# kshedden/muscato

Measured on AMD Instinct MI355X. Metric: reads/sec (100 bp, multi-map) at 1/2/4/8 MI355X; confirm-kernel HBM GB/s vs peak, higher is better.
Workload: dtype u32

## Files before the change

muscato_amd/csrc/kernels_common.hpp:

```cpp
#pragma once


#define DEV __device__ __forceinline__
#ifndef MUSC_KERNEL
#define MUSC_KERNEL __global__
#endif
#define READ_HAS_X 0x10000u

DEV uint64_t mix64(uint64_t x) {
  x ^= x >> 33;
  x *= 0xff51afd7ed558ccdULL;
  x ^= x >> 33;
  x *= 0xc4ceb9fe1a85ec53ULL;
  x ^= x >> 33;
  return x;
}

DEV uint32_t block_hash32(uint32_t k, uint32_t b) {
  uint32_t h = b ^ (k * 0x9E3779B9u + 0x7F4A7C15u);
  h ^= h >> 16;
  h *= 0x85EBCA6Bu;
  h ^= h >> 13;
  h *= 0xC2B2AE35u;
  h ^= h >> 16;
// ... 15 lines not shown
  const int nb = 2 * ww;
  uint64_t h = 0, anymask = 0, key0 = 0;
  for (int c = 0; c < nb; c += 64) {
    const int take = nb - c < 64 ? nb - c : 64;
    const uint64_t key = ext64(w, bo + c) & lowmask64(take);
    const uint64_t mk = m ? (ext64(m, bo + c) & lowmask64(take)) : 0ull;
    if (c == 0) key0 = key;
    anymask |= mk;
    h = mix64(h ^ key ^ mix64(mk + 0x9E3779B97F4A7C15ull * (uint64_t)(c + 1)));
  }
  if (direct && anymask == 0) return (uint32_t)(__brevll(key0) >> (64 - nb));
  return (uint32_t)(h >> (64 - bits));
}

DEV void block_add_u64(unsigned long long v, unsigned long long* dst) {
  __shared__ unsigned long long s_acc[16];
  for (int d = 32; d; d >>= 1) v += __shfl_xor(v, d);
  const int wid = threadIdx.x >> 6, nw = (blockDim.x + 63) >> 6;
  if ((threadIdx.x & 63) == 0) s_acc[wid] = v;
  __syncthreads();
  if (threadIdx.x == 0) {
    unsigned long long t = 0;
    for (int w = 0; w < nw; w++) t += s_acc[w];
    if (t) atomicAdd(dst, t);
  }
  __syncthreads();
}

#ifndef MAX_GRID
#define MAX_GRID 4096u
#endif

enum : int {
  CNT_ACCEPTED = 1,
  CNT_HITS = 2,
  CNT_FLAGS = 3,
  CNT_SCRATCH = 4,
  CNT_OVF_BLOCKS = 5,
  CNT_HOT = 6,
  CNT_PASS_WORDS = 8,
  CNT_BATCH = 8,
  CNT_BATCH_WORDS = 8,
  CNT_WORDS = 16,
  MB_WINDOWS = 0,
  MB_CMP = 1,
  MB_CAND = 3,
  MB_OVF = 4,
  MB_SPILL_MAX = 5,
  MB_TUPLES = 6,
  MB_STAGE_MAX = 7,
  SB_WINDOWS = 0,
  SB_CAND = 3,
  SB_PAIRS = 4,
  SB_TWO = 5,
  SB_DESC_MAX = 7,
};
constexpr unsigned long long FLAG_STAGE_OVERRUN = 1;
constexpr unsigned long long FLAG_HITS_OVERRUN = 2;
constexpr unsigned long long FLAG_SPILL_OVERRUN = 4;
constexpr unsigned long long FLAG_SPEC_REFUSED = 8;


DEV uint32_t ascii_code(unsigned char c, uint32_t* isx) {
  const uint32_t a = c == 'A', cc = c == 'C', g = c == 'G', t = c == 'T';
  *isx = !(a | cc | g | t);
  return cc | (g << 1) | (t * 3u);
}

MUSC_KERNEL void k_pack_db_ascii(const unsigned char* __restrict__ s, uint64_t nbases,
                                uint32_t* __restrict__ db2, uint32_t* __restrict__ dbm2,
                                uint64_t nwords, uint32_t* __restrict__ has_x) {
  const uint64_t w = (uint64_t)blockIdx.x * blockDim.x + threadIdx.x;
// ... 266 lines not shown
```

muscato_amd/csrc/kernels_match.hpp:

```cpp
#pragma once

#define CTX_BASES 120
#define CTX_INLINE 3
#define CTX_MAX_W 4
#define CTX_XFLAG 0x80000000u
#define CTX_XMANY 0xFFu
#define CTX_XNONE 0xFFu

struct __attribute__((aligned(128))) CtxBucket {
  uint32_t count;
  uint32_t ovf;
  uint32_t gene[CTX_INLINE];
  uint32_t jx[CTX_INLINE];
  uint32_t ctx[CTX_INLINE][8];
};
static_assert(sizeof(CtxBucket) == 128, "a context bucket is one cache line");

struct CtxEntry {
  uint32_t gene, jx;
  uint32_t ctx[8];
};
static_assert(sizeof(CtxEntry) == 40, "overflow entries are packed");

#define CTXW_BASES 200
// ... 152 lines not shown
          dst[0] = make_uint4(c[0], c[1], c[2], c[3]);
          dst[1] = make_uint4(c[4], c[5], c[6], c[7]);
        } else {
          uint32_t* p = reinterpret_cast<uint32_t*>(Ev) + ctx_entry_word<false>(T[b].ovf + (slot - CTX_INLINE));
          p[0] = gene | xgene;
          p[1] = (uint32_t)jx | xflag;
#pragma unroll
          for (int i = 0; i < 8; i++) p[2 + i] = c[i];
        }
      }
    }
  }
}

MUSC_KERNEL void k_ctx_ovf_count(const CtxBucket* __restrict__ T, uint64_t nb, uint32_t n_inline, uint64_t* __restrict__ tmp) {
  const uint64_t b = (uint64_t)blockIdx.x * blockDim.x + threadIdx.x;
  if (b < nb) {
    const uint32_t c = T[b].count;
    tmp[b] = c > n_inline ? c - n_inline : 0u;
  } else if (b == nb) {
    tmp[b] = 0;
  }
}

MUSC_KERNEL void k_ctx_ovf_set(CtxBucket* __restrict__ T, uint64_t nb, const uint64_t* __restrict__ tmp) {
  const uint64_t b = (uint64_t)blockIdx.x * blockDim.x + threadIdx.x;
  if (b < nb) T[b].ovf = (uint32_t)tmp[b];
}


struct MatchParams {
  int32_t W, ww, min_dinuc, bits, direct, mmtol, apply_mmtol, max_len, CL;
  uint32_t q1zero_mask;
  int32_t reserved0;
  int32_t win[CTX_MAX_W];
  const uint64_t* seq_off;
  const uint32_t* dbm2;
  uint32_t need[CTX_MAX_W];
  uint32_t wm[CTX_MAX_W][CTX_MAX_W][CTXW_WORDS];
  uint32_t lm[CTXW_BASES + 1][CTX_MAX_W][CTXW_WORDS];
};


inline void match_tables(MatchParams& mp) {
  for (int k = 0; k < CTX_MAX_W; k++) {
    mp.need[k] = 0;
    if (k >= mp.W) continue;
    const int sh = 2 * (mp.CL - mp.win[k]);
    mp.need[k] = ((1u << k) - 1u) | (mp.direct ? 0u : (1u << k));
    for (int kk = 0; kk < mp.W; kk++)
      for (int j = 0; j < CTXW_WORDS; j++)
        mp.wm[k][kk][j] = bit_range_mask(sh + 2 * mp.win[kk] - 32 * j, sh + 2 * (mp.win[kk] + mp.ww) - 32 * j);
    for (int len = 0; len <= CTXW_BASES; len++)
      for (int j = 0; j < CTXW_WORDS; j++) mp.lm[len][k][j] = 0x55555555u & bit_range_mask(sh - 32 * j, sh + 2 * len - 32 * j);
  }
}


#ifndef MATCH_SKETCH_BITS
#define MATCH_SKETCH_BITS 10
#endif

DEV bool ctx_fit(uint32_t jx, uint32_t rem16, int q1, int ww, int rlen, uint32_t* zflag) {
  const int left = (int)(jx > 65535u ? 65535u : jx), right = (int)rem16;
  const int tcap = left + right;
  const int lim0 = 100 - ww < tcap ? 100 - ww : tcap;
  const bool fit0 = rlen <= lim0;
  const bool inside = left == 0 ? fit0 : (rlen - q1 <= right);
  *zflag = (uint32_t)(left == q1) & (uint32_t)!fit0;
  return (q1 <= left) & inside;
}

#define REC_LEN(w) ((w) & 0xFFFFu)
#define REC_BUDGET(w) (((w) >> 17) & 0x7Fu)
#define REC_VALID(w) ((w) >> 24)
// ... 90 lines not shown
}

MUSC_KERNEL void k_xpos_check(const uint32_t* __restrict__ rd, const uint32_t* __restrict__ xpos, uint64_t nreads, int rw,
                             const uint16_t* __restrict__ nmiss_tab, uint32_t max_len, uint32_t xmax, uint32_t* __restrict__ bad) {
  const uint64_t i = (uint64_t)blockIdx.x * blockDim.x + threadIdx.x;
  if (i >= nreads) return;
  const uint32_t cnt = XPOS_CNT(xpos[i]);
  if (cnt <= xmax) return;
  const uint32_t len = rd[(i + 1) * rw - 1] & 0xFFFFu;
  const uint32_t budget = len <= max_len ? nmiss_tab[len] : 0xFFFFu;
  if (cnt == 15u || cnt <= budget) atomicOr(bad, 1u);
}

struct XWins { int32_t n, ww, q1[CTX_MAX_W]; };
template <bool WIDE>
__global__ void k_xpos_check_db(const uint32_t* __restrict__ xpos, uint64_t nreads, XWins wn, uint32_t* __restrict__ bad) {
  typedef XPos<WIDE> XP;
  const uint64_t i = (uint64_t)blockIdx.x * blockDim.x + threadIdx.x;
  if (i >= nreads) return;
  const uint32_t w = xpos[i], cnt = XPOS_CNT(w);
  if (!cnt) return;
  bool b = cnt > XP::MAX;
  for (uint32_t q = 0; q < XP::MAX && q < cnt; q++)
    for (int k = 0; k < wn.n; k++) b |= XP::at(w, q) - (uint32_t)wn.q1[k] < (uint32_t)wn.ww;
  if (b) atomicOr(bad, 1u);
}

MUSC_KERNEL __launch_bounds__(256) void k_compact_w(uint32_t nwt, const uint32_t* __restrict__ tbase,
                                                   const uint32_t* __restrict__ tcount2,
                                                   const uint32_t* __restrict__ tpre, const uint4* __restrict__ stage,
                                                   uint4* __restrict__ hits, uint64_t hits_cap,
                                                   unsigned long long* __restrict__ counters) {
  const unsigned long long base = counters[CNT_HITS];
  if (base + tpre[nwt] > hits_cap) {
    if (blockIdx.x == 0 && threadIdx.x == 0) atomicOr(&counters[CNT_FLAGS], FLAG_HITS_OVERRUN);
    return;
  }
  const uint32_t lane = threadIdx.x & 63;
  for (uint32_t wt = blockIdx.x * 4 + (threadIdx.x >> 6); wt < nwt; wt += gridDim.x * 4) {
    const uint32_t m = tcount2[wt];
    const uint4* __restrict__ src = stage + tbase[wt];
    uint4* __restrict__ dst = hits + base + tpre[wt];
    for (uint32_t j = lane; j < m; j += 64) dst[j] = src[j];
  }
}
```

muscato_amd/csrc/kernels_match_lane.hpp:

```cpp
#pragma once
#include "kernels_match_lane_inst.hpp"
#if defined(MUSC_LANE_DBG) && !defined(MUSC_LANE_DBG_SLOTS)
#define MUSC_LANE_DBG_SLOTS 3
#endif

template <int RW, int NW>
DEV void read_image_n(const Rec<RW>& rec, uint32_t sh, uint32_t (&img)[NW]) {
  const uint32_t bs = sh & 31u;
#define MUSC_IMG_W(Q) (((Q) >= 0 && (Q) < RW - 1) ? rec.w[((Q) >= 0 && (Q) < RW - 1) ? (Q) : 0] : 0u)
#define MUSC_IMG_CASE(WO)                                                  \
  case WO:                                                                 \
    _Pragma("unroll") for (int j = 0; j < NW; j++) {                       \
      const uint32_t hi = MUSC_IMG_W(j - WO), lo = MUSC_IMG_W(j - WO - 1); \
      img[j] = bs ? ((hi << bs) | (lo >> (32u - bs))) : hi;                \
    }                                                                      \
    break;
  switch (__builtin_amdgcn_readfirstlane((int)(sh >> 5))) {
    MUSC_IMG_CASE(0) MUSC_IMG_CASE(1) MUSC_IMG_CASE(2) MUSC_IMG_CASE(3)
    MUSC_IMG_CASE(4) MUSC_IMG_CASE(5) MUSC_IMG_CASE(6) MUSC_IMG_CASE(7)
    MUSC_IMG_CASE(8) MUSC_IMG_CASE(9) MUSC_IMG_CASE(10) MUSC_IMG_CASE(11) MUSC_IMG_CASE(12)
    default:
#pragma unroll
      for (int j = 0; j < NW; j++) img[j] = 0u;
      break;
// ... 44 lines not shown
  constexpr bool SPEC = SGm::on;
  static_assert(!SPEC || (SGm::nwin == W && !WIDE && XM == 0 && SGm::ww <= 15), "a specialised instance is built for its geometry's window count, 120-base buckets, no X, a direct table of one-word keys");
  constexpr int S_WW = SGm::ww, S_CL = SGm::CL, S_L = SGm::L, S_MIND = SGm::min_dinuc;
  constexpr int S_WIN[CTX_MAX_W] = {SGm::win[0], SGm::win[1], SGm::win[2], SGm::win[3]};
  if constexpr (SPEC) {
    bool same = mp->ww == S_WW && mp->CL == S_CL && mp->min_dinuc == S_MIND && mp->direct == 1 && mp->bits == 2 * S_WW && mp->W == W;
#pragma unroll
    for (int k = 0; k < W; k++) same = same && mp->win[k] == S_WIN[k] && mp->need[k] == (1u << k) - 1u;
    if (!same) {
      if (threadIdx.x == 0) atomicOr(&counters[CNT_FLAGS], FLAG_SPEC_REFUSED);
      return;
    }
  }
  const int ww = SPEC ? S_WW : mp->ww, CL = SPEC ? S_CL : mp->CL, min_dinuc = SPEC ? S_MIND : mp->min_dinuc,
            direct = SPEC ? 1 : mp->direct, bits = SPEC ? 2 * S_WW : mp->bits;
  const uint32_t q1zero = mp->q1zero_mask;
  int win[W];
#pragma unroll
  for (int k = 0; k < W; k++) win[k] = SPEC ? S_WIN[k] : mp->win[k];
  uint32_t* const s_sketch = s_dyn + 2 * NWAVE * WT * W;
  for (uint32_t t = threadIdx.x; t < CONF_NM; t += TILE) s_nm[t] = t <= (uint32_t)mp->max_len ? nmiss_tab[t] : (uint16_t)0;
  if (block_mode) {
    for (uint32_t t = threadIdx.x; t < 2u * NWAVE * WT * W; t += TILE) s_dyn[t] = 0;
    if (block_mode == 1)
      for (uint32_t t = threadIdx.x; t < (1u << MATCH_SKETCH_BITS); t += TILE) s_sketch[t] = 0;
  }
  s_best[0][threadIdx.x >> 6][threadIdx.x & 63] = 0xFFFFFFFFu;
  s_best[1][threadIdx.x >> 6][threadIdx.x & 63] = 0xFFFFFFFFu;
  if (blockIdx.x == 0 && threadIdx.x == 0) tcount2[(n + WT - 1) / WT] = 0;
  __syncthreads();

  const uint32_t nwt = (n + WT - 1) / WT;
  const uint32_t gw = blockIdx.x * NWAVE + (threadIdx.x >> 6), nw = gridDim.x * NWAVE;
  const uint64_t region = stage_cap / nw, region0 = region * gw;
  const uint64_t sregion = spill_cap / nw / 2, sregion_w = 2 * sregion * gw;
  uint64_t used = 0;
  uint32_t maxspill = 0;
  uint32_t nvalid = 0, ncand = 0, ncmp = 0, novf = 0, nrep = 0;
  const uint32_t mmtol = (uint32_t)mp->mmtol;
  const bool apply = mp->apply_mmtol != 0;

  auto fetch = [&](uint32_t wt, Rec<RW>& rec) __attribute__((always_inline)) {
    const uint32_t i = wt * WT + (opaque(threadIdx.x) & 63);
    rec.load(rd + (r0 + (i < n ? i : 0)) * (uint64_t)RW, RW);
  };
  auto phase_a = [&](uint32_t wt, const Rec<RW>& rec, uint32_t& xw, uint32_t (&bb)[W]) __attribute__((always_inline)) -> uint32_t {
    const uint32_t lane = opaque(threadIdx.x) & 63;
    const bool active = wt * WT + lane < n;
    const int len = (int)rec.len();
    uint32_t valid = 0;
    xw = 0;
    uint32_t xwin = 0;
    if constexpr (RX) {
      if (active && rec.has_x()) xw = rdx[r0 + wt * WT + lane];
      const uint32_t xc = XPOS_CNT(xw);
      if (xc > XP::MAX) xwin = 0xFFFFFFFFu;
#pragma unroll
      for (int k = 0; k < W; k++) {
        const uint32_t q1 = (uint32_t)win[k];
#pragma unroll
        for (int q = 0; q < (int)XP::MAX; q++)
          if ((uint32_t)q < xc && XP::at(xw, q) - q1 < (uint32_t)ww) xwin |= 1u << k;
      }
    }
    if (ww <= 16 && direct) {
      const uint32_t kmask = ww == 16 ? 0xFFFFFFFFu : ((1u << (2 * ww)) - 1u);
#pragma unroll
      for (int k = 0; k < W; k++) {
        const uint32_t q1 = (uint32_t)win[k], q2 = q1 + (uint32_t)ww;
// ... 189 lines not shown
  for (int k = 0; k < W; k++) wc_prev[k] = oc_prev[k] = ovf_prev[k] = 0, bb_prev[k] = WB_NONE;
  uint32_t o_n = 0, o_k = 0, o_seg = 0, o_meta = 0, o_xw = 0;
  Rec<RW> o_rec;
  o_rec.zero();
  u32x4_u o_q[NQ];
  uint32_t o_t[NT];
#pragma unroll
  for (int q = 0; q < NQ; q++) o_q[q] = u32x4_u{0, 0, 0, 0};
#pragma unroll
  for (int q = 0; q < NT; q++) o_t[q] = 0;

  auto rec_of = [&](uint32_t p, uint32_t seg, Rec<RW>& rec) __attribute__((always_inline)) {
    const uint32_t wid = opaque(threadIdx.x) >> 6;
    const uint4* src = reinterpret_cast<const uint4*>(&s_rec[p][wid][seg * RW]);
#pragma unroll
    for (int q = 0; q < RW / 4; q++) {
      const uint4 v = src[q];
      rec.w[4 * q] = v.x; rec.w[4 * q + 1] = v.y; rec.w[4 * q + 2] = v.z; rec.w[4 * q + 3] = v.w;
    }
  };

  auto phase_a_all = [&](uint32_t wt, uint32_t p, const Rec<RW>& rec, uint32_t& meta, uint32_t& xw, uint32_t (&bb)[W]) __attribute__((always_inline)) {
    const uint32_t tid = opaque(threadIdx.x);
    const uint32_t lane = tid & 63, wid = tid >> 6;
    const uint32_t valid = phase_a(wt, rec, xw, bb);
    const uint32_t len = rec.len();
    const uint32_t budget0 = len < CONF_NM ? s_nm[len] : 0u;
    meta = len | ((budget0 > 127u ? 127u : budget0) << 17) | (valid << 24);
    uint4* dst = reinterpret_cast<uint4*>(&s_rec[p][wid][lane * RW]);
#pragma unroll
    for (int q = 0; q < RW / 4; q++) dst[q] = make_uint4(rec.w[4 * q], rec.w[4 * q + 1], rec.w[4 * q + 2], rec.w[4 * q + 3]);
  };

  if (gw < nwt) {
    Rec<RW> rec0;
    fetch(gw, rec0);
    phase_a_all(gw, 0, rec0, meta_cur, xw_cur, bb_cur);
    if (gw + nw < nwt) fetch(gw + nw, rec_nx);
    wave_lds_sync();
    issue_window(bb_cur[0], va, vb);
  }
  uint32_t wt = gw;
  bool have_prev = false;
#ifdef MUSC_LANE_PROF
  unsigned long long pf[12] = {0, 0, 0, 0, 0, 0, 0, 0, 0, 0, 0, 0}, pt0 = __builtin_amdgcn_s_memtime(), pstart = pt0;
  uint32_t pf_tiles = 0;
#define PF(i) { const unsigned long long t_ = __builtin_amdgcn_s_memtime(); pf[i] += t_ - pt0; pt0 = t_; }
#elif defined(MUSC_LANE_MARK)
#define PF(i) asm volatile("; MARK " #i);
#else
#define PF(i)
#endif
  while (wt < nwt || have_prev) {
    const bool have_cur = wt < nwt;
    const uint32_t tid = opaque(threadIdx.x);
    const uint32_t lane = tid & 63, wid = tid >> 6;
    uint32_t* const cnt_l = s_cb[wid];
    uint32_t* const base_l = s_cb[wid] + WT;
    uint4* const line_l = s_line[wid];
    const bool have_next = wt + nw < nwt;

    auto report_any = [&](uint32_t p, uint32_t& nl, uint32_t w, uint32_t gene, uint32_t pos) __attribute__((always_inline)) {
      const bool acc = w != NX_REJECT;
      if (acc && block_mode) atomicAdd(&s_dyn[(p * NWAVE + wid) * WT * W + ((w >> 20) & 15u) * WT + (w >> 24)], 1u);
      const bool rep = acc && !(w & NX_DUP);
      const unsigned long long vote = __ballot(rep);
      if (vote == 0) return;
      const uint32_t below = __builtin_amdgcn_mbcnt_hi((uint32_t)(vote >> 32), __builtin_amdgcn_mbcnt_lo((uint32_t)vote, 0u));
      const uint32_t slot = nl + below;
      nl += (uint32_t)__popcll(vote);
      if (!rep) return;
      atomicMin(&s_best[p][wid][w >> 24], w & 0xFFFFu);
      if (slot < WLIST) {
        s_list[p][wid][slot] = make_uint3(w, gene, pos);
      } else if (slot - WLIST < sregion) {
        spill[sregion_w + p * sregion + (slot - WLIST)] = make_uint4(w, gene, pos, 0u);
      }
    };
    auto entry_compare = [&](uint32_t p, uint32_t& nl, uint32_t ul, uint32_t n_items, uint32_t ek, uint32_t seg, uint32_t meta,
                             uint32_t xw, const Rec<RW>& rec, const u32x4_u (&eq)[NQ], const uint32_t (&et)[NT]) __attribute__((always_inline)) {
#ifdef MUSC_LANE_DBG
      if (MUSC_LANE_DBG & 32) return;
#endif
      const bool have = lane < n_items;
      if (!__any(have)) return;
      const int len = (int)REC_LEN(meta);
      const uint32_t xi = DBX && (eq[0].y & CTX_XFLAG) ? 0x100u | (eq[0].x >> 24) : 0u;
      const uint32_t gene = xi ? eq[0].x & 0xFFFFFFu : eq[0].x, jx = DBX ? eq[0].y & ~CTX_XFLAG : eq[0].y;
      uint32_t c[NW];
#pragma unroll
      for (int j = 0; j < NW; j++) {
        const int wi = j + 2;
        c[j] = wi < 4 * NQ ? (wi % 4 == 0 ? eq[wi / 4].x : wi % 4 == 1 ? eq[wi / 4].y : wi % 4 == 2 ? eq[wi / 4].z : eq[wi / 4].w) : et[wi - 4 * NQ];
// ... 175 lines not shown
        const uint32_t* sp = reinterpret_cast<const uint32_t*>(spill + sregion_w + pp * sregion + (j - WLIST));
        *gene = __hip_atomic_load(sp + 1, __ATOMIC_RELAXED, __HIP_MEMORY_SCOPE_AGENT);
        *pos = __hip_atomic_load(sp + 2, __ATOMIC_RELAXED, __HIP_MEMORY_SCOPE_AGENT);
        return __hip_atomic_load(sp, __ATOMIC_RELAXED, __HIP_MEMORY_SCOPE_AGENT);
      };
      const uint32_t nuse = spill_ok ? nl : (nl < WLIST ? nl : WLIST);
      uint32_t kw = NX_REJECT, kg = 0, kp = 0, ko = 0;
      if (nuse) {
        best_l[lane] = bestr;
        cnt_l[lane] = 0;
        wave_lds_sync();
        if (lane < nuse) {
          const uint32_t w = item(lane, &kg, &kp);
          const uint32_t rl = w >> 24;
          const uint32_t thr = apply ? best_l[rl] + mmtol : 0xFFFFu;
          if ((w & 0xFFFFu) <= thr) {
            kw = w;
            ko = atomicAdd(&cnt_l[rl], 1u);
          }
        }
        for (uint32_t j = 64 + lane; j < nuse; j += 64) {
          uint32_t g, p;
          const uint32_t w = item(j, &g, &p);
          const uint32_t rl = w >> 24;
          const uint32_t thr = apply ? best_l[rl] + mmtol : 0xFFFFu;
          if ((w & 0xFFFFu) <= thr) atomicAdd(&cnt_l[rl], 1u);
        }
        wave_lds_sync();
        cnum += cnt_l[lane];
      }
      const uint32_t inc = wave_scan_incl(cnum);
      const uint32_t total = __builtin_amdgcn_readlane(inc, 63);
      const uint32_t mybase = inc - cnum;
      const uint64_t base = region0 + used;
      const bool fits = spill_ok && used + total <= region;
      if (lane == 0) {
        tbase[wt_prev] = (uint32_t)base;
        tcount2[wt_prev] = fits ? total : 0u;
      }
      if (fits && total) {
        const uint32_t rid = (uint32_t)(r0 + wt_prev * WT + lane);
        if (s0) put_tuple(&stage[base + mybase], rid, k0g_prev, k0p_prev, k0w_prev & 0xFFFFu);
        if (s1) put_tuple(&stage[base + mybase + (s0 ? 1u : 0u)], rid, k1g_prev, k1p_prev, k1w_prev & 0xFFFFu);
        if (nuse) {
          base_l[lane] = mybase + nown;
          wave_lds_sync();
          if (kw != NX_REJECT) {
            const uint32_t rl = kw >> 24;
            put_tuple(&stage[base + base_l[rl] + ko], (uint32_t)(r0 + wt_prev * WT + rl), kg, kp, kw & 0xFFFFu);
          }
          if (nuse > 64) {
            for (uint32_t j = 64 + lane; j < nuse; j += 64) {
              uint32_t g, p;
              const uint32_t w = item(j, &g, &p);
              const uint32_t rl = w >> 24, v = w & 0xFFFFu;
              const uint32_t thr = apply ? best_l[rl] + mmtol : 0xFFFFu;
              if (v > thr) continue;
              const uint32_t ord = atomicAdd(&cnt_l[rl], 0xFFFFFFFFu) - 1u;
              put_tuple(&stage[base + base_l[rl] + ord], (uint32_t)(r0 + wt_prev * WT + rl), g, p, v);
            }
          }
        }
      }
      wave_lds_sync();
      best_l[lane] = 0xFFFFFFFFu;
      used += total;
      nrep += kc_prev < (uint32_t)OWNK ? kc_prev : (uint32_t)OWNK;
      nrep += lane == 0 ? nl : 0u;
// ... 30 lines not shown
        const bool acc = w != NX_REJECT;
        wck += acc ? 1u : 0u;
        const bool rep = acc && !(w & NX_DUP);
        const bool first = OWNK >= 1 && rep && kc == 0, second = OWNK >= 2 && rep && kc == 1, later = rep && kc >= (uint32_t)OWNK;
        k0w = first ? w : k0w; k0g = first ? gene : k0g; k0p = first ? pos : k0p;
        k1w = second ? w : k1w; k1g = second ? gene : k1g; k1p = second ? pos : k1p;
        kc += rep ? 1u : 0u;
        const uint32_t v = w & 0xFFFFu;
        best = rep && v < best ? v : best;
        const unsigned long long vote = __ballot(later);
        if (vote == 0) return;
        const uint32_t below = __builtin_amdgcn_mbcnt_hi((uint32_t)(vote >> 32), __builtin_amdgcn_mbcnt_lo((uint32_t)vote, 0u));
        const uint32_t slot = nlist + below;
        nlist += (uint32_t)__popcll(vote);
        if (!later) return;
        if (slot < WLIST) {
          list_cur[slot] = make_uint3(w, gene, pos);
        } else if (slot - WLIST < sregion) {
          spill[sregion_w + par * sregion + (slot - WLIST)] = make_uint4(w, gene, pos, 0u);
        }
      };

      auto window = [&](auto kc) __attribute__((always_inline)) {
        constexpr int k = decltype(kc)::value;
        const int q1 = win[k];
        const uint32_t sh = 2u * (uint32_t)(CL - q1);
        WinTab tb;
        win_tab(ulen, k, sh, (uint32_t)rlen, tb);
        {
#pragma unroll
          for (int i = 0; i < 8; i++) line_l[i * 64 + lane] = i < 4 ? va[i] : vb[i - 4];
        }
        PF(0)
        if (k == 0 && have_prev) entry_fetch();
        if (W == 1) {
          if (have_prev) finish_prev();
          if (have_next) phase_a_all(wt + nw, par ^ 1u, rec_nx, meta_nx, xw_nx, bb_nx);
          wave_lds_sync();
        }
        if (k + 1 < W) {
          issue_window(bb_cur[k + 1 < W ? k + 1 : 0], va, vb);
        } else {
          if (have_next) issue_window(bb_nx[0], va, vb);
          if (wt + 2 * nw < nwt) fetch(wt + 2 * nw, rec_nx);
        }
        PF(1)
        wave_lds_sync();
        const uint32_t rb = lane * 8u + (((lane >> 1) & 7u) ^ (lane & 1u));
        const uint4 h0 = line_l[rb], h1 = line_l[rb ^ 1u];
        const uint32_t cnt = bb_cur[k] != WB_NONE ? h0.x : 0u;
        ncand += cnt;
        oc[k] = cnt > (uint32_t)NIN ? cnt - (uint32_t)NIN : 0u;
        ovf[k] = h0.y;
        novf += oc[k];
        PF(2)
        if (W > 1 && k == 0 && have_next) phase_a_all(wt + nw, par ^ 1u, rec_nx, meta_nx, xw_nx, bb_nx);
        PF(8)
        if (W > 1 && k == 1 && have_prev) finish_prev();
        if (k + 1 == W) {
          uint32_t pre[W], total = 0;
#pragma unroll
          for (int kk = 0; kk < W; kk++) {
            const uint32_t inc = wave_scan_incl(oc[kk]);
            pre[kk] = total + inc - oc[kk];
            total += (uint32_t)__builtin_amdgcn_readlane((int)inc, 63);
          }
#ifdef MUSC_LANE_DBG
          if (MUSC_LANE_DBG & 4) total = 0;
#endif
          total_cur = total;
          owner_tables(0, oc, ovf, pre);
          o_n = total < (uint32_t)WT ? total : (uint32_t)WT;
          const uint32_t probe = lane < o_n ? (uint32_t)s_own[wid][lane] : 0u;
          o_k = probe >> 6;
          o_seg = probe & 63u;
          o_meta = s_meta[par][wid][o_seg];
          if constexpr (RX) o_xw = s_xp[par][wid][o_seg];
          rec_of(par, o_seg, o_rec);
        }
        wave_lds_sync();
        PF(3)
        uint32_t img[NW], xm[NW];
        {
          Rec<RW> rec;
          rec_of(par, lane, rec);
          read_image_n<RW, NW>(rec, sh, img);
        }
        x_mask(xw_cur, sh, xm);
        if constexpr (!WIDE) {
// ... 55 lines not shown
      if constexpr (W > 2) window(std::integral_constant<int, 2>{});
      if constexpr (W > 3) window(std::integral_constant<int, 3>{});
#ifdef MUSC_LANE_PROF
      pf_tiles++;
#endif
    } else {
      entry_fetch();
      finish_prev();
    }
    wave_lds_sync();
    have_prev = have_cur;
    if (have_cur) {
      wt_prev = wt;
      nlist_prev = nlist;
      best_prev = best;
      kc_prev = kc; k0w_prev = k0w; k0g_prev = k0g; k0p_prev = k0p; k1w_prev = k1w; k1g_prev = k1g; k1p_prev = k1p;
      ulen_prev = ulen;
      total_prev = total_cur;
#pragma unroll
      for (int k = 0; k < W; k++) {
        if constexpr (BB_LDS) {
          const uint32_t ln = opaque(threadIdx.x) & 63;
          s_bbp[wid][k][ln] = bb_cur[k];
          if (block_mode) s_dyn[(par * NWAVE + wid) * WT * W + k * WT + ln] += wc[k];
        } else {
          bb_prev[k] = bb_cur[k];
          wc_prev[k] = wc[k];
        }
        bb_cur[k] = bb_nx[k], oc_prev[k] = oc[k], ovf_prev[k] = ovf[k];
      }
      meta_cur = meta_nx;
      xw_cur = xw_nx;
      par ^= 1u;
      wt += nw;
    }
    wave_lds_sync();
    PF(5)
  }
#ifdef MUSC_LANE_PROF
  if ((gw % 37) == 0 && (threadIdx.x & 63) == 0 && pf_tiles > 4) printf("fin %u %u %llu %llu\n", gw, pf_tiles, pstart, (unsigned long long)__builtin_amdgcn_s_memtime());
  if ((gw == 0 || gw == 1001) && (threadIdx.x & 63) == 0 && pf_tiles > 4)
    printf("wave %u: %u tiles, cycles/tile: total %llu | arrive(wait+lds write) %llu issue %llu hdr %llu phA %llu finish_prev(epass %llu rest+phD %llu) expand %llu img %llu slots %llu end %llu\n", gw, pf_tiles,
           (__builtin_amdgcn_s_memtime() - pstart) / pf_tiles, pf[0] / pf_tiles, pf[1] / pf_tiles, pf[2] / pf_tiles, pf[8] / pf_tiles,
           pf[6] / pf_tiles, pf[7] / pf_tiles, pf[3] / pf_tiles, pf[9] / pf_tiles, pf[4] / pf_tiles, pf[5] / pf_tiles);
#endif
  {
    __shared__ unsigned long long s_red[NWAVE][8];
    unsigned long long v[5] = {nvalid, ncmp, ncand, novf, nrep};
#pragma unroll
    for (int q = 0; q < 5; q++)
      for (int d = 32; d; d >>= 1) v[q] += __shfl_xor(v[q], d);
    const uint32_t wv = threadIdx.x >> 6;
    if ((threadIdx.x & 63) == 0) {
#pragma unroll
      for (int q = 0; q < 5; q++) s_red[wv][q] = v[q];
      s_red[wv][5] = used <= region ? used : 0;
      s_red[wv][6] = used;
      s_red[wv][7] = ((unsigned long long)(used > region) << 32) | maxspill;
    }
    __syncthreads();
    if (threadIdx.x == 0) {
      unsigned long long t[6] = {0, 0, 0, 0, 0, 0}, mx_used = 0, mx_spill = 0, over = 0;
      for (int w = 0; w < NWAVE; w++) {
        for (int q = 0; q < 6; q++) t[q] += s_red[w][q];
        mx_used = s_red[w][6] > mx_used ? s_red[w][6] : mx_used;
        const unsigned long long sp = s_red[w][7] & 0xFFFFFFFFull;
        mx_spill = sp > mx_spill ? sp : mx_spill;
        over |= s_red[w][7] >> 32;
      }
      if (t[0]) atomicAdd(&counters[CNT_BATCH + MB_WINDOWS], t[0]);
      if (t[1]) atomicAdd(&counters[CNT_BATCH + MB_CMP], t[1]);
      if (t[2]) atomicAdd(&counters[CNT_BATCH + MB_CAND], t[2]);
      if (t[3]) atomicAdd(&counters[CNT_BATCH + MB_OVF], t[3]);
      if (t[4]) atomicAdd(&counters[CNT_ACCEPTED], t[4]);
      if (t[5]) atomicAdd(&counters[CNT_BATCH + MB_TUPLES], t[5]);
      atomicMax(&counters[CNT_BATCH + MB_STAGE_MAX], mx_used);
      if (mx_spill) atomicMax(&counters[CNT_BATCH + MB_SPILL_MAX], mx_spill);
      if (over) atomicOr(&counters[CNT_FLAGS], FLAG_STAGE_OVERRUN);
      if (mx_spill > sregion) atomicOr(&counters[CNT_FLAGS], FLAG_SPILL_OVERRUN);
    }
  }
  if (block_mode == 1) {
    __syncthreads();
    uint32_t hot = 0;
    for (uint32_t t = threadIdx.x; t < (1u << MATCH_SKETCH_BITS); t += TILE) hot |= s_sketch[t] >= block_thr;
    if (__any(hot) && (threadIdx.x & 63) == 0) atomicOr(&counters[CNT_HOT], 1ull);
  }
}
```

muscato_amd/csrc/kernels_match_lane_inst.hpp:

```cpp
#pragma once
#ifndef MATCHT_WAVES
#define MATCHT_WAVES 2
#endif
#ifndef MATCHT_WLIST
#define MATCHT_WLIST 96
#endif
template <int SG>
struct SpecGeom {
  static constexpr bool on = false;
  static constexpr int ww = 0, CL = 0, L = 0, min_dinuc = 0, nwin = 0;
  static constexpr int win[CTX_MAX_W] = {0, 0, 0, 0};
};
template <>
struct SpecGeom<1> {
  static constexpr bool on = true;
  static constexpr int ww = 15, CL = 20, L = 100, min_dinuc = 5, nwin = 2;
  static constexpr int win[CTX_MAX_W] = {0, 20, 0, 0};
};
#define MUSC_SPEC_GEOMS 1

#define MUSC_MATCH_ARGS                                                                                              \
  (const uint32_t*, uint64_t, uint32_t, const MatchParams*, const uint16_t*, const CtxBucket*, const CtxEntry*, uint4*, \
   uint64_t, uint4*, uint64_t, uint32_t*, uint32_t*, int, uint32_t, uint32_t*, unsigned long long*, const uint32_t*)
typedef void (*match_kernel_t) MUSC_MATCH_ARGS;

template <int RW, int W, int XM, bool WIDE, int SG>
__global__ __launch_bounds__(TILE, MATCHT_WAVES) void k_match_t(const uint32_t* __restrict__ rd, uint64_t r0, uint32_t n,
                                                                const MatchParams* __restrict__ mp,
                                                                const uint16_t* __restrict__ nmiss_tab,
                                                                const CtxBucket* __restrict__ T, const CtxEntry* __restrict__ E,
                                                                uint4* __restrict__ stage, uint64_t stage_cap,
                                                                uint4* __restrict__ spill, uint64_t spill_cap,
                                                                uint32_t* __restrict__ tbase, uint32_t* __restrict__ tcount2,
                                                                int block_mode, uint32_t block_thr,
                                                                uint32_t* __restrict__ block_table,
                                                                unsigned long long* __restrict__ counters,
                                                                const uint32_t* __restrict__ rdx);
#ifndef MATCHG_WAVES_OF
// ... 44 lines not shown
```

muscato_amd/csrc/muscato_hip.hip:

```cpp

#include <hip/hip_runtime.h>
#include <rccl/rccl.h>
#include <dlfcn.h>

#include <algorithm>
#include <cstdarg>
#include <cstdio>
#include <cstdlib>
#include <cstring>
#include <map>
#include <mutex>
#include <string>
#include <type_traits>
#include <vector>

#include "../../include/muscato_hip.h"

#include "kernels_common.hpp"
#include "kernels_index.hpp"
#include "kernels_screen.hpp"
#include "kernels_confirm.hpp"
#include "kernels_match.hpp"
#include "kernels_match_lane_inst.hpp"
#include "kernels_screen_lane.hpp"
// ... 95 lines not shown
  void release() {
    for (int i = 0; i < n; i++) (void)hipFree(p[i]);
    n = 0;
  }
  ~TmpBufs() { release(); }
};

}

struct StreamPlan {
  std::vector<uint64_t> piece_end, batch_end;
};
static void stream_plan(uint64_t nreads, uint64_t batch_reads, StreamPlan* sp) {
  auto up64 = [](uint64_t x) { return (x + 63) & ~63ull; };
  sp->piece_end.clear();
  sp->batch_end.clear();
  const uint64_t full = std::max<uint64_t>(up64(batch_reads), 64);
  const uint64_t last_max = std::max<uint64_t>(up64(batch_reads / 16), 64);
  const uint64_t piece = up64(std::max<uint64_t>(batch_reads / 4, 64));
  for (uint64_t r0 = 0; r0 < nreads;) {
    const uint64_t left = nreads - r0;
    const uint64_t n = left >= 2 * full ? full : left <= last_max ? left : up64((left + 1) / 2);
    for (uint64_t p = r0 + piece; p < r0 + n; p += piece) sp->piece_end.push_back(p);
    r0 += n;
    sp->piece_end.push_back(r0);
    sp->batch_end.push_back(r0);
  }
}
static uint64_t stream_plan_batch(const StreamPlan& sp, uint64_t r0) {
  const auto it = std::upper_bound(sp.batch_end.begin(), sp.batch_end.end(), r0);
  return it == sp.batch_end.end() ? 0 : *it - r0;
}

struct EnvKnobs {
  enum { IDX_AUTO = 0, IDX_CLASSIC, IDX_LINES, IDX_CLASSIC64 };
  int index = IDX_AUTO;
  bool match_dma = false;
  bool screen_wg = false;
  int context = 0;
  bool no_x_context = false;
  bool force_wide = false;
  int index_bits = 0;
  bool ctx_direct = false;
  int debug_grid = 0;
  bool debug_sync = false;
  int graph = -1;
  bool pipeline = false;
  bool no_spec = false;
  long batch_reads = 0;
  long index_budget_mb = 0;
  uint64_t stage_bytes = 64ull << 20;
  uint64_t stage_lines = 1ull << 20;
  void read() {
    *this = EnvKnobs();
    auto is = [](const char* v, const char* w) { return v && !strcmp(v, w); };
    const char* e = getenv("MUSC_INDEX");
    index = is(e, "classic") ? IDX_CLASSIC : is(e, "lines") ? IDX_LINES : is(e, "classic64") ? IDX_CLASSIC64 : IDX_AUTO;
    e = getenv("MUSC_MATCH");
    match_dma = is(e, "dma");
    screen_wg = is(getenv("MUSC_SCREEN"), "wg");
    e = getenv("MUSC_CONTEXT");
    context = is(e, "narrow") ? 1 : is(e, "wide") ? 2 : 0;
    no_x_context = getenv("MUSC_NO_X_CONTEXT") != nullptr;
    force_wide = getenv("MUSC_DEBUG_FORCE_WIDE") != nullptr;
    if ((e = getenv("MUSC_DEBUG_INDEX_BITS"))) index_bits = atoi(e);
    ctx_direct = (e = getenv("MUSC_DEBUG_CTX_DIRECT")) && atoi(e) > 0;
    if ((e = getenv("MUSC_DEBUG_GRID"))) debug_grid = atoi(e);
    debug_sync = getenv("MUSC_DEBUG_SYNC") != nullptr;
    if ((e = getenv("MUSC_GRAPH"))) graph = atoi(e);
    if ((e = getenv("MUSC_PIPELINE"))) pipeline = atoi(e) > 0;
    no_spec = getenv("MUSC_NO_SPEC") != nullptr;
    if ((e = getenv("MUSC_BATCH_READS"))) batch_reads = atol(e);
    if ((e = getenv("MUSC_DEBUG_INDEX_BUDGET_MB"))) index_budget_mb = atol(e);
    if ((e = getenv("MUSC_DEBUG_STAGE_BYTES")) && atoll(e) > 0) stage_bytes = (uint64_t)atoll(e);
    if ((e = getenv("MUSC_DEBUG_STAGE_LINES")) && atoll(e) > 0) stage_lines = (uint64_t)atoll(e);
  }
};

struct musc_ctx {
  int device = 0;
  hipStream_t stream = nullptr;
  std::string err;
  EnvKnobs env;

  uint32_t* db2 = nullptr;
  uint32_t* dbm2 = nullptr;
  bool db_has_x = false;
  bool reads_have_x = false;
  DevBuf<uint32_t> rdx;
  uint64_t rdx_epoch = ~0ull;
  int rdx_wide = -1;
  uint64_t xok_epoch = ~0ull;
  double xok_pmatch = -1.0;
  int32_t xok_mmp1 = -1;
  bool xok = false;
  uint32_t* dbx = nullptr;
  uint64_t max_tlen = 0;
  uint64_t xokdb_epoch = ~0ull;
  int32_t xokdb_key[CTX_MAX_W + 3] = {0};
  bool xokdb = false;
  uint64_t* seq_off = nullptr;
  uint32_t nseq = 0;
  uint64_t nbases = 0;
  uint64_t db_words = 0;
// ... 1940 lines not shown
```

muscato_amd/csrc/muscato_pass.hpp:

```cpp
#pragma once

namespace {

bool screen_lane(const musc_ctx* c, bool mask) {
  return c->idx_lines && !mask && !c->rdm && (c->rw == 4 || c->rw == 8 || c->rw == 12 || c->rw == 16) && !c->env.screen_wg;
}

template <class F>
auto by_rw(int rw, F&& f) {
  switch (rw) {
    case 4: return f(std::integral_constant<int, 4>{});
    case 8: return f(std::integral_constant<int, 8>{});
    case 12: return f(std::integral_constant<int, 12>{});
    case 16: return f(std::integral_constant<int, 16>{});
    default: return f(std::integral_constant<int, 0>{});
  }
}

typedef decltype(&k_screen_t<8>) screen_t_fn;
typedef decltype(&k_screen<0, false, false, false>) screen_fn;
typedef decltype(&k_confirm<0, false, false>) confirm_fn;
template <class Fn>
struct Inst {
  Fn fn;
// ... 174 lines not shown
}

static void launch_match(musc_ctx* c, const PassPlan& pl, uint64_t r0, uint32_t n, unsigned ngrid) {
  const size_t lds = match_dyn_lds(match_kind(c, pl.pp.W), pl.pp.W, pl.block_mode);
  const uint32_t* const rdx = c->reads_have_x ? (const uint32_t*)c->rdx.p : (const uint32_t*)nullptr;
  hipLaunchKernelGGL(pl.kern, dim3(ngrid), dim3(TILE), lds, c->stream, c->rd, r0, n, c->d_mp, c->nmiss_tab.p, c->ctx_T,
                     c->ctx_E, c->stage.p, c->stage.cap, c->spill.p, c->spill.cap, c->bs[0].tbase.p, c->tcount2.p,
                     pl.block_mode, pl.block_thr, c->block_table.p, c->counters, rdx);
}

template <int SG>
static bool spec_geom_equals(const MatchParams& mp) {
  typedef SpecGeom<SG> G;
  if (mp.W != G::nwin || mp.ww != G::ww || mp.CL != G::CL || mp.min_dinuc != G::min_dinuc || mp.direct != 1 || mp.bits != 2 * G::ww) return false;
  for (int k = 0; k < G::nwin; k++)
    if (mp.win[k] != G::win[k] || mp.need[k] != (1u << k) - 1u) return false;
  return true;
}
static int spec_geom_matches(const musc_ctx* c, const MatchParams& mp) {
  if (c->env.no_spec) return 0;
  if (c->rw != 8 || c->idx_wide || c->db_has_x || c->reads_have_x) return 0;
  return spec_geom_equals<1>(mp) ? 1 : 0;
}

static int match_setup(musc_ctx* c, PassPlan* pl) {
  const PathParams& pp = pl->pp;
  if (c->rw != 4 && c->rw != 8 && c->rw != 12 && !(c->rw == 16 && c->idx_wide))
    return fail(c, 12, "internal: record stride %d on the context path", c->rw);
  static thread_local MatchParams mp;
  memset(&mp, 0, sizeof mp);
  mp.W = pp.W; mp.ww = pp.ww; mp.min_dinuc = pp.min_dinuc; mp.bits = pp.bits; mp.direct = pp.direct;
  mp.mmtol = pp.mmtol; mp.apply_mmtol = pp.apply_mmtol; mp.max_len = pp.max_len; mp.CL = c->idx_CL;
  mp.q1zero_mask = pp.q1zero_mask;
  mp.seq_off = c->db_has_x ? c->seq_off : nullptr;
  mp.dbm2 = c->db_has_x ? c->dbm2 : nullptr;
  for (int k = 0; k < pp.W && k < CTX_MAX_W; k++) mp.win[k] = pp.win[k];
  match_tables(mp);
  c->spec_geom = spec_geom_matches(c, mp);
  c->stats.match_variant = (match_kind(c, pp.W) == MK_DMA ? 4u : 2u) + (c->spec_geom ? 1u : 0u);
  if (!c->h_mp_valid || memcmp(&mp, &c->h_mp, sizeof mp) != 0) {
    c->h_mp = mp;
    HIPCHK(c, hipMemcpyAsync(c->d_mp, &c->h_mp, sizeof mp, hipMemcpyHostToDevice, c->stream));
    HIPCHK(c, hipStreamSynchronize(c->stream));
    c->h_mp_valid = true;
  }
  const int xm = c->db_has_x ? 2 : c->reads_have_x ? 1 : 0;
  const MatchInst inst = match_instance(match_kind(c, pp.W), c->spec_geom, c->rw, c->idx_wide != 0, pp.W, xm);
  pl->kern = inst.fn;
  c->last_inst[0] = inst.id;
  if (!pl->kern) return fail(c, 12, "internal: no fused kernel instance for record stride %d, %d windows", c->rw, pp.W);
  pl->resident = match_resident(c, pl->kern, pp.W, pl->block_mode);
  return 0;
}

static int pass_setup(musc_ctx* c, const musc_params* P, PassPlan* pl, BatchCursor* cur) {
  int rc = 0;
  const float keep_index_ms = c->stats.ms_index_build;
  memset(&c->stats, 0, sizeof c->stats);
  c->stats.ms_index_build = keep_index_ms;
  c->stats.n_reads = c->nreads;
  c->nhits = 0;

  pl->P = P;
  PathParams& pp = pl->pp;
  memset(&pp, 0, sizeof pp);
  pp.W = P->n_windows;
// ... 185 lines not shown
    if (!clk.ev0 || !clk.ev1) return fail(c, 10, "hipEventCreate failed");
    const bool replay = use_graph && c->graph_exec && c->graph_epoch == c->data_epoch && c->graph_block_mode == pl.block_mode &&
                        memcmp(&c->graph_params, pl.P, sizeof *pl.P) == 0;
    const bool capture = use_graph && !replay;
    if (capture && c->graph_exec) {
      (void)hipGraphExecDestroy(c->graph_exec);
      c->graph_exec = nullptr;
    }
    clk.tm.off = capture || replay;
    CaptureGuard cap;
    if (capture) {
      if (cap.begin(c->stream) != hipSuccess) {
        (void)hipGetLastError();
        *what = PASS_RERUN_NO_GRAPH;
        return 0;
      }
    } else if (!replay) {
      HIPCHK(c, hipEventRecord(clk.ev0, c->stream));
    }
    uint64_t tot[CNT_BATCH_WORDS] = {0}, r0 = 0;
    c->stats.n_batches = c->stats.match_launches = 0;
    bool again = false;
    if (!replay) {
      HIPCHK(c, hipMemsetAsync(c->counters, 0, CNT_WORDS * sizeof(unsigned long long), c->stream));
      if (pl.block_mode == 2) HIPCHK(c, hipMemsetAsync(c->block_table.p, 0, (1ull << BLOCK_TABLE_BITS) * 4, c->stream));
    }
    while (!replay && r0 < c->nreads) {
      const uint32_t n = cur.reads_at(r0, c->nreads);
      const uint32_t ntiles = nblk(n, WT);
      const uint64_t sgrid = std::min<uint64_t>(nblk(n, TILE), pl.resident);
      const uint64_t swaves = sgrid * (TILE / 64);
      if (!sized) {
        if ((rc = ensure_tiles(c, c->bs[0], ntiles)) ||
            (rc = ensure(c, c->stage, std::max<uint64_t>(FIRST_PASS_TUPLES_PER_READ * n, swaves * 64))) ||
            (rc = ensure(c, c->spill, swaves * 32)))
          return rc;
        HIPCHK(c, hipMemsetAsync(c->counters + CNT_BATCH, 0, CNT_BATCH_WORDS * sizeof(unsigned long long), c->stream));
      }
      if ((rc = upload_prepare(c, r0, n, c->stream))) return rc;
      clk.tm.begin(0);
      {
        Range rg("k_match");
        launch_match(c, pl, r0, n, (unsigned)sgrid);
      }
      HIPCHK(c, hipGetLastError());
      clk.tm.end(0);
      c->stats.match_launches++;
      c->stats.n_batches++;
      if (!sized) {
        if ((rc = pass_peek(c))) return rc;
        const uint64_t* h = c->h_pinned;
        const uint64_t need_stage = h[CNT_BATCH + MB_STAGE_MAX] * swaves, need_spill = 2 * h[CNT_BATCH + MB_SPILL_MAX] * swaves;
        if (need_stage > BATCH_OFFSET_CAP) {
          if (n == 1) return fail(c, 6, "one read has %llu tuples (> 2^31)", (unsigned long long)h[CNT_BATCH + MB_STAGE_MAX]);
          cur.halve(n);
          again = true;
          break;
        }
        if (h[CNT_FLAGS] & FLAG_SPEC_REFUSED)
          return fail(c, 12, "internal: the kernel instance specialised for geometry %d refused this run's parameters", c->spec_geom);
        if (h[CNT_FLAGS] || need_stage > c->stage.cap || need_spill > c->spill.cap) {
          if (need_stage > c->stage.cap && (rc = ensure(c, c->stage, need_stage + need_stage / 4 + swaves))) return rc;
          if (need_spill > c->spill.cap && (rc = ensure(c, c->spill, need_spill + need_spill / 4 + swaves))) return rc;
          again = true;
          break;
        }
        for (int i = 0; i < CNT_BATCH_WORDS; i++) tot[i] += h[CNT_BATCH + i];
        if ((rc = ensure(c, c->hits, h[CNT_HITS] + h[CNT_BATCH + MB_TUPLES], true))) return rc;
      }
      Range rgc("scan + k_compact_w");
      const dim3 cgrid(std::min(nblk(ntiles, 4), 4u * MAX_GRID));
      if ((rc = launch_compact(c, clk.tm, k_compact_w, cgrid, ntiles, c->bs[0].tbase.p, c->stream))) return rc;
      r0 += n;
    }
    if (again) continue;
    if (!replay && (rc = pass_close(c, pl, capture ? nullptr : clk.ev1))) return rc;
    if (capture) {
      hipGraph_t g = nullptr;
      hipError_t ge = cap.end(&g);
      if (ge == hipSuccess) ge = hipGraphInstantiate(&c->graph_exec, g, nullptr, nullptr, 0);
      if (g) (void)hipGraphDestroy(g);
      if (ge != hipSuccess) {
        (void)hipGetLastError();
        c->graph_exec = nullptr;
        *what = PASS_RERUN_NO_GRAPH;
        return 0;
      }
      c->graph_epoch = c->data_epoch;
      c->graph_params = *pl.P;
      c->graph_block_mode = pl.block_mode;
      c->graph_batches = c->stats.n_batches;
    }
    if (capture || replay) {
      c->stats.n_batches = c->stats.match_launches = c->graph_batches;
      HIPCHK(c, hipEventRecord(clk.ev0, c->stream));
// ... 166 lines not shown
```

Baseline: 2.102 billion.

## Add ticket-based wave-tile scheduling and shared stage overflow pool

Adds an optional dynamic scheduler in which waves claim groups of wave-tiles through an atomic ticket counter instead of a fixed stride, to balance uneven per-read work. It also reserves a shared pool at the end of the stage buffer that waves fall back to via an atomic when their private region overflows, so a single heavy wave no longer forces a buffer regrow and batch rerun. The host sizing logic is reworked to account for the pool. Tickets are off by default; the pool path is always active, at the cost of extra atomics and a smaller per-wave region.

```diff
diff --git a/muscato_amd/csrc/kernels_common.hpp b/muscato_amd/csrc/kernels_common.hpp
--- a/muscato_amd/csrc/kernels_common.hpp
+++ b/muscato_amd/csrc/kernels_common.hpp
@@ -71,12 +71,14 @@
 #endif
 
 enum : int {
+  CNT_TICKET = 0,
   CNT_ACCEPTED = 1,
   CNT_HITS = 2,
   CNT_FLAGS = 3,
   CNT_SCRATCH = 4,
   CNT_OVF_BLOCKS = 5,
   CNT_HOT = 6,
+  CNT_POOL = 7,
   CNT_PASS_WORDS = 8,
   CNT_BATCH = 8,
   CNT_BATCH_WORDS = 8,
diff --git a/muscato_amd/csrc/kernels_match.hpp b/muscato_amd/csrc/kernels_match.hpp
--- a/muscato_amd/csrc/kernels_match.hpp
+++ b/muscato_amd/csrc/kernels_match.hpp
@@ -208,7 +208,7 @@
 struct MatchParams {
   int32_t W, ww, min_dinuc, bits, direct, mmtol, apply_mmtol, max_len, CL;
   uint32_t q1zero_mask;
-  int32_t reserved0;
+  int32_t sched;
   int32_t win[CTX_MAX_W];
   const uint64_t* seq_off;
   const uint32_t* dbm2;
@@ -217,6 +217,18 @@
   uint32_t lm[CTXW_BASES + 1][CTX_MAX_W][CTXW_WORDS];
 };
 
+
+constexpr int32_t SCHED_TICKETS = 1;
+constexpr int32_t SCHED_NO_REGION = 2;
+
+constexpr uint64_t STAGE_POOL_SMALL = 1ull << 16;
+__host__ __device__ inline uint64_t stage_pool(uint64_t stage_cap) {
+  const uint64_t half = stage_cap / 2, small = half < STAGE_POOL_SMALL ? half : STAGE_POOL_SMALL, eighth = stage_cap / 8;
+  return eighth > small ? eighth : small;
+}
+inline uint64_t stage_with_pool(uint64_t regions) {
+  return regions <= STAGE_POOL_SMALL ? 2 * regions : regions <= 7 * STAGE_POOL_SMALL ? regions + STAGE_POOL_SMALL : regions + regions / 7 + 8;
+}
 
 inline void match_tables(MatchParams& mp) {
   for (int k = 0; k < CTX_MAX_W; k++) {
@@ -373,6 +385,7 @@
                                                    uint4* __restrict__ hits, uint64_t hits_cap,
                                                    unsigned long long* __restrict__ counters) {
   const unsigned long long base = counters[CNT_HITS];
+  if (blockIdx.x == 0 && threadIdx.x == 0) counters[CNT_TICKET] = counters[CNT_POOL] = 0;
   if (base + tpre[nwt] > hits_cap) {
     if (blockIdx.x == 0 && threadIdx.x == 0) atomicOr(&counters[CNT_FLAGS], FLAG_HITS_OVERRUN);
     return;
diff --git a/muscato_amd/csrc/kernels_match_lane.hpp b/muscato_amd/csrc/kernels_match_lane.hpp
--- a/muscato_amd/csrc/kernels_match_lane.hpp
+++ b/muscato_amd/csrc/kernels_match_lane.hpp
@@ -100,9 +100,13 @@
 
   const uint32_t nwt = (n + WT - 1) / WT;
   const uint32_t gw = blockIdx.x * NWAVE + (threadIdx.x >> 6), nw = gridDim.x * NWAVE;
-  const uint64_t region = stage_cap / nw, region0 = region * gw;
+  const bool tickets = (mp->sched & SCHED_TICKETS) != 0;
+  const uint64_t pool_cap = stage_pool(stage_cap), pool0 = stage_cap - pool_cap;
+  const uint64_t region = (mp->sched & SCHED_NO_REGION) ? 0 : pool0 / nw, region0 = region * gw;
   const uint64_t sregion = spill_cap / nw / 2, sregion_w = 2 * sregion * gw;
   uint64_t used = 0;
+  uint64_t used_r = 0, staged = 0;
+  bool pool_full = false;
   uint32_t maxspill = 0;
   uint32_t nvalid = 0, ncand = 0, ncmp = 0, novf = 0, nrep = 0;
   const uint32_t mmtol = (uint32_t)mp->mmtol;
@@ -358,15 +362,33 @@
     for (int q = 0; q < RW / 4; q++) dst[q] = make_uint4(rec.w[4 * q], rec.w[4 * q + 1], rec.w[4 * q + 2], rec.w[4 * q + 3]);
   };
 
-  if (gw < nwt) {
+  constexpr uint32_t TG = MATCHT_TICKET_G;
+  static_assert(TG >= 1 && (TG & (TG - 1)) == 0, "a ticket stands for a power of two of wave-tiles");
+  const uint32_t gwu = (uint32_t)__builtin_amdgcn_readfirstlane((int)gw);
+  uint32_t tk_draw = 0;
+  auto tk_succ = [&](uint32_t last) __attribute__((always_inline)) -> uint32_t {
+    if (last >= nwt) return 0xFFFFFFFFu;
+    if ((last + 1) & (TG - 1)) return last + 1;
+    if (last / TG == gwu) return (gwu + nw) * TG;
+    return (2 * nw + (uint32_t)__builtin_amdgcn_readfirstlane((int)tk_draw)) * TG;
+  };
+  auto tk_issue = [&](uint32_t last) __attribute__((always_inline)) {
+    if (tickets && last < nwt && !((last + 1) & (TG - 1)) && last / TG != gwu) {
+      if ((opaque(threadIdx.x) & 63) == 0)
+        tk_draw = __builtin_amdgcn_atomic_inc32(reinterpret_cast<uint32_t*>(&counters[CNT_TICKET]), 0xFFFFFFFFu, __ATOMIC_RELAXED, "agent");
+    }
+  };
+  uint32_t wt = tickets ? gwu * TG : gwu;
+  uint32_t wt_nx = (uint32_t)__builtin_amdgcn_readfirstlane((int)(tickets ? tk_succ(wt) : wt + nw)), wt_nx2 = 0xFFFFFFFFu;
+  if (wt < nwt) {
     Rec<RW> rec0;
-    fetch(gw, rec0);
-    phase_a_all(gw, 0, rec0, meta_cur, xw_cur, bb_cur);
-    if (gw + nw < nwt) fetch(gw + nw, rec_nx);
+    fetch(wt, rec0);
+    phase_a_all(wt, 0, rec0, meta_cur, xw_cur, bb_cur);
+    if (wt_nx < nwt) fetch(wt_nx, rec_nx);
+    tk_issue(wt_nx);
     wave_lds_sync();
     issue_window(bb_cur[0], va, vb);
   }
-  uint32_t wt = gw;
   bool have_prev = false;
 #ifdef MUSC_LANE_PROF
   unsigned long long pf[12] = {0, 0, 0, 0, 0, 0, 0, 0, 0, 0, 0, 0}, pt0 = __builtin_amdgcn_s_memtime(), pstart = pt0;
@@ -384,7 +406,7 @@
     uint32_t* const cnt_l = s_cb[wid];
     uint32_t* const base_l = s_cb[wid] + WT;
     uint4* const line_l = s_line[wid];
-    const bool have_next = wt + nw < nwt;
+    const bool have_next = wt_nx < nwt;
 
     auto report_any = [&](uint32_t p, uint32_t& nl, uint32_t w, uint32_t gene, uint32_t pos) __attribute__((always_inline)) {
       const bool acc = w != NX_REJECT;
@@ -626,8 +648,19 @@
       const uint32_t inc = wave_scan_incl(cnum);
       const uint32_t total = __builtin_amdgcn_readlane(inc, 63);
       const uint32_t mybase = inc - cnum;
-      const uint64_t base = region0 + used;
-      const bool fits = spill_ok && used + total <= region;
+      uint64_t base = region0 + used_r;
+      bool fits = spill_ok;
+      if (used_r + total <= region) {
+        used_r += total;
+      } else if (spill_ok) {
+        unsigned long long at = 0;
+        if (lane == 0) at = atomicAdd(&counters[CNT_POOL], (unsigned long long)total);
+        at = ((unsigned long long)(uint32_t)__builtin_amdgcn_readfirstlane((int)(at >> 32)) << 32) | (uint32_t)__builtin_amdgcn_readfirstlane((int)(uint32_t)at);
+        fits = at + total <= pool_cap;
+        pool_full = pool_full || !fits;
+        base = pool0 + at;
+      }
+      if (fits) staged += total;
       if (lane == 0) {
         tbase[wt_prev] = (uint32_t)base;
         tcount2[wt_prev] = fits ? total : 0u;
@@ -724,17 +757,19 @@
           for (int i = 0; i < 8; i++) line_l[i * 64 + lane] = i < 4 ? va[i] : vb[i - 4];
         }
         PF(0)
+        if (k == 0) wt_nx2 = (uint32_t)__builtin_amdgcn_readfirstlane((int)(tickets ? tk_succ(wt_nx) : wt_nx + nw));
         if (k == 0 && have_prev) entry_fetch();
         if (W == 1) {
           if (have_prev) finish_prev();
-          if (have_next) phase_a_all(wt + nw, par ^ 1u, rec_nx, meta_nx, xw_nx, bb_nx);
+          if (have_next) phase_a_all(wt_nx, par ^ 1u, rec_nx, meta_nx, xw_nx, bb_nx);
           wave_lds_sync();
         }
         if (k + 1 < W) {
           issue_window(bb_cur[k + 1 < W ? k + 1 : 0], va, vb);
         } else {
           if (have_next) issue_window(bb_nx[0], va, vb);
-          if (wt + 2 * nw < nwt) fetch(wt + 2 * nw, rec_nx);
+          if (wt_nx2 < nwt) fetch(wt_nx2, rec_nx);
+          tk_issue(wt_nx2);
         }
         PF(1)
         wave_lds_sync();
@@ -746,7 +781,7 @@
         ovf[k] = h0.y;
         novf += oc[k];
         PF(2)
-        if (W > 1 && k == 0 && have_next) phase_a_all(wt + nw, par ^ 1u, rec_nx, meta_nx, xw_nx, bb_nx);
+        if (W > 1 && k == 0 && have_next) phase_a_all(wt_nx, par ^ 1u, rec_nx, meta_nx, xw_nx, bb_nx);
         PF(8)
         if (W > 1 && k == 1 && have_prev) finish_prev();
         if (k + 1 == W) {
@@ -868,7 +903,8 @@
       meta_cur = meta_nx;
       xw_cur = xw_nx;
       par ^= 1u;
-      wt += nw;
+      wt = wt_nx;
+      wt_nx = wt_nx2;
     }
     wave_lds_sync();
     PF(5)
@@ -890,9 +926,9 @@
     if ((threadIdx.x & 63) == 0) {
 #pragma unroll
       for (int q = 0; q < 5; q++) s_red[wv][q] = v[q];
-      s_red[wv][5] = used <= region ? used : 0;
+      s_red[wv][5] = staged;
       s_red[wv][6] = used;
-      s_red[wv][7] = ((unsigned long long)(used > region) << 32) | maxspill;
+      s_red[wv][7] = ((unsigned long long)pool_full << 32) | maxspill;
     }
     __syncthreads();
     if (threadIdx.x == 0) {
diff --git a/muscato_amd/csrc/kernels_match_lane_inst.hpp b/muscato_amd/csrc/kernels_match_lane_inst.hpp
--- a/muscato_amd/csrc/kernels_match_lane_inst.hpp
+++ b/muscato_amd/csrc/kernels_match_lane_inst.hpp
@@ -4,6 +4,9 @@
 #endif
 #ifndef MATCHT_WLIST
 #define MATCHT_WLIST 96
+#endif
+#ifndef MATCHT_TICKET_G
+#define MATCHT_TICKET_G 4
 #endif
 template <int SG>
 struct SpecGeom {
diff --git a/muscato_amd/csrc/muscato_hip.hip b/muscato_amd/csrc/muscato_hip.hip
--- a/muscato_amd/csrc/muscato_hip.hip
+++ b/muscato_amd/csrc/muscato_hip.hip
@@ -151,6 +151,9 @@
   return it == sp.batch_end.end() ? 0 : *it - r0;
 }
 
+#ifndef MUSC_TILES_DEFAULT_TICKET
+#define MUSC_TILES_DEFAULT_TICKET false
+#endif
 struct EnvKnobs {
   enum { IDX_AUTO = 0, IDX_CLASSIC, IDX_LINES, IDX_CLASSIC64 };
   int index = IDX_AUTO;
@@ -166,6 +169,8 @@
   int graph = -1;
   bool pipeline = false;
   bool no_spec = false;
+  bool tile_tickets = MUSC_TILES_DEFAULT_TICKET;
+  bool no_stage_region = false;
   long batch_reads = 0;
   long index_budget_mb = 0;
   uint64_t stage_bytes = 64ull << 20;
@@ -189,6 +194,9 @@
     if ((e = getenv("MUSC_GRAPH"))) graph = atoi(e);
     if ((e = getenv("MUSC_PIPELINE"))) pipeline = atoi(e) > 0;
     no_spec = getenv("MUSC_NO_SPEC") != nullptr;
+    e = getenv("MUSC_TILES");
+    tile_tickets = is(e, "ticket") ? true : is(e, "static") ? false : tile_tickets;
+    no_stage_region = is(getenv("MUSC_DEBUG_STAGE_REGION"), "0");
     if ((e = getenv("MUSC_BATCH_READS"))) batch_reads = atol(e);
     if ((e = getenv("MUSC_DEBUG_INDEX_BUDGET_MB"))) index_budget_mb = atol(e);
     if ((e = getenv("MUSC_DEBUG_STAGE_BYTES")) && atoll(e) > 0) stage_bytes = (uint64_t)atoll(e);
diff --git a/muscato_amd/csrc/muscato_pass.hpp b/muscato_amd/csrc/muscato_pass.hpp
--- a/muscato_amd/csrc/muscato_pass.hpp
+++ b/muscato_amd/csrc/muscato_pass.hpp
@@ -230,6 +230,7 @@
   mp.W = pp.W; mp.ww = pp.ww; mp.min_dinuc = pp.min_dinuc; mp.bits = pp.bits; mp.direct = pp.direct;
   mp.mmtol = pp.mmtol; mp.apply_mmtol = pp.apply_mmtol; mp.max_len = pp.max_len; mp.CL = c->idx_CL;
   mp.q1zero_mask = pp.q1zero_mask;
+  mp.sched = (c->env.tile_tickets ? SCHED_TICKETS : 0) | (c->env.no_stage_region ? SCHED_NO_REGION : 0);
   mp.seq_off = c->db_has_x ? c->seq_off : nullptr;
   mp.dbm2 = c->db_has_x ? c->dbm2 : nullptr;
   for (int k = 0; k < pp.W && k < CTX_MAX_W; k++) mp.win[k] = pp.win[k];
@@ -481,7 +482,7 @@
       const uint64_t swaves = sgrid * (TILE / 64);
       if (!sized) {
         if ((rc = ensure_tiles(c, c->bs[0], ntiles)) ||
-            (rc = ensure(c, c->stage, std::max<uint64_t>(FIRST_PASS_TUPLES_PER_READ * n, swaves * 64))) ||
+            (rc = ensure(c, c->stage, stage_with_pool(std::max<uint64_t>(FIRST_PASS_TUPLES_PER_READ * n, swaves * 64)))) ||
             (rc = ensure(c, c->spill, swaves * 32)))
           return rc;
         HIPCHK(c, hipMemsetAsync(c->counters + CNT_BATCH, 0, CNT_BATCH_WORDS * sizeof(unsigned long long), c->stream));
@@ -499,8 +500,14 @@
       if (!sized) {
         if ((rc = pass_peek(c))) return rc;
         const uint64_t* h = c->h_pinned;
-        const uint64_t need_stage = h[CNT_BATCH + MB_STAGE_MAX] * swaves, need_spill = 2 * h[CNT_BATCH + MB_SPILL_MAX] * swaves;
-        if (need_stage > BATCH_OFFSET_CAP) {
+        const uint64_t region = c->env.no_stage_region ? 0 : (c->stage.cap - stage_pool(c->stage.cap)) / swaves;
+        const bool pool_out = (h[CNT_FLAGS] & FLAG_STAGE_OVERRUN) != 0;
+        const bool grow_stage = pool_out || (!c->env.no_stage_region && h[CNT_BATCH + MB_STAGE_MAX] > region);
+        uint64_t need_stage = c->env.no_stage_region ? 0 : h[CNT_BATCH + MB_STAGE_MAX] * swaves;
+        need_stage = stage_with_pool(need_stage + need_stage / 4 + swaves);
+        if (pool_out) need_stage = std::max(need_stage, 2 * c->stage.cap);
+        const uint64_t need_spill = 2 * h[CNT_BATCH + MB_SPILL_MAX] * swaves;
+        if (grow_stage && need_stage > BATCH_OFFSET_CAP) {
           if (n == 1) return fail(c, 6, "one read has %llu tuples (> 2^31)", (unsigned long long)h[CNT_BATCH + MB_STAGE_MAX]);
           cur.halve(n);
           again = true;
@@ -508,8 +515,8 @@
         }
         if (h[CNT_FLAGS] & FLAG_SPEC_REFUSED)
           return fail(c, 12, "internal: the kernel instance specialised for geometry %d refused this run's parameters", c->spec_geom);
-        if (h[CNT_FLAGS] || need_stage > c->stage.cap || need_spill > c->spill.cap) {
-          if (need_stage > c->stage.cap && (rc = ensure(c, c->stage, need_stage + need_stage / 4 + swaves))) return rc;
+        if (h[CNT_FLAGS] || grow_stage || need_spill > c->spill.cap) {
+          if (grow_stage && need_stage > c->stage.cap && (rc = ensure(c, c->stage, need_stage))) return rc;
           if (need_spill > c->spill.cap && (rc = ensure(c, c->spill, need_spill + need_spill / 4 + swaves))) return rc;
           again = true;
           break;
```

Measured after the change: 2.095 billion. No clear change (-0.3%).
